# SinclaM/ray-tracer-challenge

Measured on AMD Instinct MI355X. Metric: Mrays/sec (primary+secondary), scenes/cover.json 1920x1080 depth 5, higher is better.
Workload: dtype f64

## Files before the change

ray-tracer-challenge_amd/csrc/rtc_capi.hip:

```cpp
#include <algorithm>
#include <chrono>
#include <atomic>
#include <cmath>
#include <cstdarg>
#include <cstdio>
#include <cstddef>
#include <cstring>
#include <memory>
#include <string>
#include <thread>
#include <unordered_set>
#include <vector>

#include "../../include/rtc.h"
#include "../../include/rtc_diag.h"
#include <sched.h>
#include <sys/mman.h>
#include <unistd.h>

#include "rtc_device.h"

extern "C" __global__ void rtc_scatter_tiles_kernel(const double* tiles, const uint32_t* tile_list, const uint32_t n_tiles, const uint32_t tile_w,
                                                    const uint32_t tile_h, const uint32_t hsize, const uint32_t vsize, double* canvas);
extern "C" __global__ void rtc_scatter_tiles_rgba8_kernel(const double* tiles, const uint32_t* tile_list, const uint32_t n_tiles,
// ... 226 lines not shown
  if (map.n_chunks >= min_chunks) return true;
  return simple3Trial(s, map) && threeWaves(s);
}

bool tablesInLds(const rtc_scene* s) {
  return s->dev.n_roots <= RTC_LDS_ROOTS && s->dev.n_materials <= RTC_LDS_MATERIALS &&
         s->dev.n_patterns <= RTC_LDS_PATTERNS && s->dev.n_lights <= RTC_LDS_LIGHTS;
}

struct KernelChoice {
  decltype(&rtc_render_kernel) fn;
  const char* name;
  decltype(&rtc_render_kernel_area) area = nullptr;
  decltype(&rtc_render_kernel_ms) ms = nullptr;
  decltype(&rtc_render_kernel_area_ms) area_ms = nullptr;
  KernelChoice(decltype(&rtc_render_kernel) f, const char* n) : fn(f), name(n) {}
  KernelChoice(decltype(&rtc_render_kernel_area) a, const char* n) : fn(nullptr), name(n), area(a) {}
  KernelChoice(decltype(&rtc_render_kernel_ms) m, const char* n) : fn(nullptr), name(n), ms(m) {}
  KernelChoice(decltype(&rtc_render_kernel_area_ms) am, const char* n) : fn(nullptr), name(n), area_ms(am) {}
  void launch(uint32_t blocks, hipStream_t stream, const rtc_scene* s, const DevScene& dev, const DevCamera& cam, const DevPixelMap& map,
              uint32_t max_depth, double* d_out, DevStats* st_now, DevStats* st_next) const {
    DevSampling smp = s->sampling;
    smp.pixel_base = static_cast<unsigned long long>(smp.sample_base) * (static_cast<unsigned long long>(cam.hsize) * cam.vsize);
    if (area_ms)
      hipLaunchKernelGGL(area_ms, dim3(blocks), dim3(256), 0, stream, dev, cam, map, max_depth, d_out, st_now, st_next, s->area, smp);
    else if (ms)
      hipLaunchKernelGGL(ms, dim3(blocks), dim3(256), 0, stream, dev, cam, map, max_depth, d_out, st_now, st_next, smp);
    else if (area)
      hipLaunchKernelGGL(area, dim3(blocks), dim3(256), 0, stream, dev, cam, map, max_depth, d_out, st_now, st_next, s->area);
    else
      hipLaunchKernelGGL(fn, dim3(blocks), dim3(256), 0, stream, dev, cam, map, max_depth, d_out, st_now, st_next);
  }
};
bool samplingKernels(const rtc_scene* s) { return s->sampling_on || s->sample_pass != 0u || rtcOptions().sampling_kernels != 0.0; }
#define RTC_KERNEL(k) KernelChoice{k, #k}
bool usesGeneral3(const rtc_scene* s) {
#if RTC_BVH8
  if (!s->general3_ok) return false;
  const double forced = rtcOptions().waves3;
  if (forced >= 0.0) return forced != 0.0;
  return threeWaves(s);
#else
  (void)s;
  return false;
#endif
}
KernelChoice ldsKernel(const rtc_scene* s, const DevPixelMap& map) {
  if (usesSimple3(s, map)) return s->box_cull ? RTC_KERNEL(rtc_render_kernel_simple3_b) : RTC_KERNEL(rtc_render_kernel_simple3);
#if RTC_BVH8
  if (usesGeneral3(s)) return RTC_KERNEL(rtc_render_kernel3);
#endif
  if (s->simple_kernel)
    return s->ext_kernel ? RTC_KERNEL(rtc_render_kernel_simple_ext) : (s->box_cull ? RTC_KERNEL(rtc_render_kernel_simple_b) : RTC_KERNEL(rtc_render_kernel_simple));
  if (s->flat_kernel) return s->ext_kernel ? RTC_KERNEL(rtc_render_kernel_flat_ext) : RTC_KERNEL(rtc_render_kernel_flat);
// ... 2572 lines not shown
```

ray-tracer-challenge_amd/csrc/rtc_device.h:

```cpp
#pragma once
#include <hip/hip_runtime.h>
#include <stdint.h>

#define RTC_NODE_BIT 0x80000000u
#define RTC_NO_LEAF 0xFFFFFFFFu
#define RTC_NO_ITEM 0xFFFFFFFFu
#define RTC_PACKET_ITEMS 16u
#define RTC_ITEM_MAX_CHUNKS 0x100000u

#ifndef RTC_TRAV_STACK
#define RTC_TRAV_STACK 64
#endif
#ifndef RTC_LDS_TRAV
#define RTC_LDS_TRAV 8
#endif
#ifndef RTC_MAX_DEPTH
#define RTC_MAX_DEPTH 16
#endif
#define RTC_RAY_STACK (RTC_MAX_DEPTH + 2)

struct DevMaterial {
  double ambient, diffuse, specular, shininess, reflective, transparency, ior;
  uint32_t pattern;
  uint32_t shininess_int;
// ... 209 lines not shown
};

struct DevPixelMap {
  uint32_t mode;
  uint32_t x0, y0, w, h;
  uint32_t tile_w, tile_h, first_tile, tile_stride, n_my_tiles;
  uint32_t tiles_x;
  uint32_t chunks_x;
  uint32_t chunks_per_region;
  uint32_t n_chunks;
  const uint32_t* __restrict__ tile_list;
  uint32_t n_units;
  const uint32_t* __restrict__ order;
  const uint32_t* __restrict__ n_units_dev;
  uint32_t* __restrict__ cost;
  uint32_t* __restrict__ packet_time;
  PendingRec* __restrict__ ray_stack;
  uint32_t ray_stack_levels;
#ifdef RTC_PROFILE
  uint32_t ray_stack_waves;
#endif
  uint32_t pull_min_idle;
  uint32_t row_packets;
};

struct DevChunkShape {
  float rays;
  float depth;
  uint32_t parts;
  uint8_t q[16];
};

struct DevSchedInfo {
  uint32_t n_units;
  uint32_t heaviest;
  uint32_t pad_[2];
  unsigned long long total;
};

#define RTC_PACK_CLASSES 136
struct DevPackState {
  uint32_t cnt[RTC_PACK_CLASSES];
  uint32_t cursor[RTC_PACK_CLASSES];
  unsigned long long total;
  uint32_t heaviest;
  uint32_t parts_cursor;
// ... 34 lines not shown
```

ray-tracer-challenge_amd/csrc/rtc_kernels.hip:

```cpp
#include "rtc_device.h"

#include <type_traits>

#if defined(RTC_PROFILE) && defined(RTC_PROFILE_LITE)
#define RTC_STAMP(sec)                                                     \
  do {                                                                     \
    if ((sec) == 7) prof_t = __builtin_amdgcn_s_memtime();                 \
    (void)prof_sec;                                                        \
  } while (0)
#define RTC_COUNT(slot) do { } while (0)
#define RTC_HIST_BEGIN() do { } while (0)
#define RTC_HIST_END(kind) do { } while (0)
#elif defined(RTC_PROFILE)
#define RTC_STAMP(sec)                                                     \
  do {                                                                     \
    const unsigned long long now_ = __builtin_amdgcn_s_memtime();          \
    prof_acc[prof_sec] += now_ - prof_t;                                   \
    prof_t = now_;                                                         \
    prof_sec = (sec);                                                      \
  } while (0)
#define RTC_COUNT(slot)                                                                 \
  do {                                                                                  \
    prof2[slot] += 1ull;                                                                \
    prof2[(slot) + 1] += static_cast<unsigned long long>(__builtin_popcountll(__ballot(true))); \
// ... 1863 lines not shown
  } else {
    pix_x = row_pt(cam.inv + 0, world_x, world_y, -1.0);
    pix_y = row_pt(cam.inv + 4, world_x, world_y, -1.0);
    pix_z = row_pt(cam.inv + 8, world_x, world_y, -1.0);
    r.ox = row_pt(cam.inv + 0, 0.0, 0.0, 0.0);
    r.oy = row_pt(cam.inv + 4, 0.0, 0.0, 0.0);
    r.oz = row_pt(cam.inv + 8, 0.0, 0.0, 0.0);
  }
  double dx = pix_x - r.ox, dy = pix_y - r.oy, dz = pix_z - r.oz;
  const double mag = __builtin_sqrt((dx * dx + dy * dy) + dz * dz);
  if (mag != 0.0) {
    dx = dx / mag;
    dy = dy / mag;
    dz = dz / mag;
  }
  r.dx = dx;
  r.dy = dy;
  r.dz = dz;
  return r;
}
#define RTC_SAMPLE_MASK 0xFFFFu
#define RTC_SAMPLE_OWNER 0x10000u

}

template <bool LDS, bool CSG, int WORLD = 0, int WAVES = 2, bool COOP = false, bool BOX = true, bool AREA = false, bool MS = false>
__device__ __forceinline__ void render_body(const DevScene& S, const DevCamera& cam, const DevPixelMap& map,
                                            const uint32_t max_depth, double* __restrict__ out,
                                            DevStats* __restrict__ stats, DevStats* __restrict__ next_stats,
                                            const DevAreaLights& area = DevAreaLights{}, const DevSampling& smp = DevSampling{}) {
  static_assert(!AREA || !COOP, "the area kernels run no cooperative iterations");
  static_assert(!MS || !COOP, "the sampling kernels run no cooperative iterations");
  RTC_PRIO_PHASE(RTC_PRIO_WORK);
#ifndef RTC_PROFILE
  if (blockIdx.x == 0u) {
    uint32_t* z = reinterpret_cast<uint32_t*>(next_stats);
    for (uint32_t i = threadIdx.x; i < sizeof(DevStats) / sizeof(uint32_t); i += blockDim.x) z[i] = 0u;
  }
#else
  (void)next_stats;
  if (threadIdx.x == 0u) rtc_prof_stats = stats;
#ifndef RTC_PROFILE_LITE
  if (threadIdx.x < 160u) rtc_prof_counts[threadIdx.x / 40u][threadIdx.x % 40u] = 0ull;
#endif
  __syncthreads();
#endif
// ... 82 lines not shown
    __syncthreads();
    recs = lds_recs;
    cull.sphere = lds_cull;
    cull.box = lds_box;
    mats = lds_mat;
    pats = lds_pat;
    lights = lds_light;
  }
#ifdef RTC_PROFILE
  if (!LDS) {
    if (threadIdx.x == 0u) {
      rtc_oob_avail[0] = S.n_root_recs;
      rtc_oob_avail[1] = S.n_root_cull;
      rtc_oob_avail[2] = S.n_root_box;
      rtc_oob_avail[3] = S.n_materials;
      rtc_oob_avail[4] = S.n_patterns;
      rtc_oob_avail[5] = 6u * S.n_lights;
    }
    __syncthreads();
  }
  const size_t out_extent = map.mode == 0u ? static_cast<size_t>(map.w) * map.h : static_cast<size_t>(map.n_my_tiles) * map.tile_w * map.tile_h;
  const bool stack_ok = (static_cast<size_t>(blockIdx.x) * 4u + (threadIdx.x >> 6)) < map.ray_stack_waves;
#endif
  const uint32_t lane = threadIdx.x & 63u;
  const unsigned long long lanes_below = (1ull << lane) - 1ull;
  auto bits_below = [&](unsigned long long m) -> uint32_t { return static_cast<uint32_t>(__builtin_popcountll(m & lanes_below)); };

  uint32_t items = RTC_NO_ITEM, item_next = RTC_PACKET_ITEMS;
  uint32_t pk_cur = RTC_NO_ITEM;
  unsigned long long pk_t0 = 0ull;
  const uint32_t n_units = map.n_units_dev != nullptr ? __builtin_amdgcn_readfirstlane(*map.n_units_dev) : map.n_units;
  uint32_t chunk_pos = 64u, chunk_end = 64u;
  uint32_t chunk_rx0 = 0u, chunk_ry0 = 0u, chunk_px0 = 0u, chunk_py0 = 0u, chunk_w = 0u, chunk_h = 0u;
  size_t chunk_out0 = 0;
  bool drained = false;
  bool first_pull = true;

  bool has_pixel = false, have_cur = false;
  bool shared = false;
  size_t out_index = 0;
  uint32_t share_rays = 0u;
  double* const acc = lds_acc[threadIdx.x >> 6][threadIdx.x & 63u];
  uint32_t* const trav_stack = FLAT ? nullptr : &lds_trav[threadIdx.x >> 6][0][(RTC_BVH8 ? 2u : 1u) * (threadIdx.x & 63u)];
  acc[0] = acc[1] = acc[2] = 0.0;
  uint32_t* samp_word = nullptr;
  if constexpr (MS) {
// ... 42 lines not shown
  const unsigned long long prof_real0 = __builtin_amdgcn_s_memrealtime();
  unsigned long long prof_real_fetch = prof_real0;
#endif
  for (;;) {
    RTC_STAMP(0);
    RTC_PRIO_PHASE(RTC_PRIO_DEAL);
    bool next_sample = false;
    if (!have_cur) {
      if (sp > base) {
        cur = load_level(--sp, lane);
        have_cur = true;
      } else {
        sp = base = 0;
        if constexpr (MS) {
          if (has_pixel) {
            const uint32_t w = *samp_word;
            if ((w & RTC_SAMPLE_OWNER) != 0u && (w & RTC_SAMPLE_MASK) + 1u < smp.samples) {
              *samp_word = w + 1u;
              next_sample = true;
            }
          }
        }
        if (!next_sample && has_pixel && RTC_IN_BOUNDS(RTC_OOB_CANVAS, out_index < out_extent)) {
          double* __restrict__ o = out + 3 * out_index;
          const double acc_r = acc[0], acc_g = acc[1], acc_b = acc[2];
          if (!shared) {
            typedef double Double2 __attribute__((ext_vector_type(2), aligned(8)));
            Double2 rg;
            rg.x = acc_r;
            rg.y = acc_g;
            __builtin_nontemporal_store(rg, reinterpret_cast<Double2*>(o));
            __builtin_nontemporal_store(acc_b, o + 2);
          } else
          {
            atomicAdd(o + 0, acc_r);
            atomicAdd(o + 1, acc_g);
            atomicAdd(o + 2, acc_b);
          }
          if (map.cost != nullptr) {
            if (!shared) {
              map.cost[out_index] = share_rays;
            } else {
              atomicAdd(map.cost + out_index, share_rays);
            }
          }
          share_rays = 0u;
          has_pixel = false;
        }
#ifdef RTC_PROFILE
        else if (has_pixel && !next_sample) {
          share_rays = 0u;
          has_pixel = false;
        }
#endif
      }
    }
    RTC_STAMP(8);
    {
      const bool idle = !have_cur && !next_sample;
      const bool donor = have_cur && sp > base;
      const unsigned long long imask = __ballot(idle), dmask = __ballot(donor);
      if (imask != 0ull && dmask != 0ull) {
        const uint32_t pairs = min(static_cast<uint32_t>(__builtin_popcountll(imask)),
                                   static_cast<uint32_t>(__builtin_popcountll(dmask)));
        const uint32_t irank = bits_below(imask);
        const uint32_t drank = bits_below(dmask);
        if (donor && drank < pairs) {
          mailbox[drank] = uint4{MS ? lane | (*samp_word & RTC_SAMPLE_MASK) << 8 : lane, static_cast<uint32_t>(base++), static_cast<uint32_t>(out_index), static_cast<uint32_t>(out_index >> 32)};
          if (!shared && RTC_IN_BOUNDS(RTC_OOB_CANVAS, out_index < out_extent)) {
            double* __restrict__ o = out + 3 * out_index;
            o[0] = 0.0;
            o[1] = 0.0;
            o[2] = 0.0;
            if (map.cost != nullptr) map.cost[out_index] = 0u;
            __builtin_amdgcn_fence(__ATOMIC_RELEASE, "workgroup");
          }
          shared = true;
        }
        __builtin_amdgcn_fence(__ATOMIC_RELEASE, "wavefront");
        __builtin_amdgcn_wave_barrier();
        __builtin_amdgcn_fence(__ATOMIC_ACQUIRE, "wavefront");
        if (idle && irank < pairs) {
          const uint4 m = mailbox[irank];
          cur = load_level(static_cast<int>(m.y), MS ? m.x & 63u : m.x);
          if constexpr (MS) *samp_word = m.x >> 8;
          out_index = static_cast<size_t>(m.z) | (static_cast<size_t>(m.w) << 32);
          have_cur = true;
          has_pixel = true;
          shared = true;
          acc[0] = acc[1] = acc[2] = 0.0;
          n_stolen++;
        }
        if (sp == base) sp = base = 0;
      }
    }
    RTC_STAMP(9);
    bool want = !have_cur && !next_sample, got_pixel = false;
    uint32_t new_px = 0u, new_py = 0u;
    unsigned long long wmask = __ballot(want);
    while (wmask) {
      if (chunk_pos >= chunk_end) {
        uint32_t unit = RTC_NO_ITEM;
        if (item_next < RTC_PACKET_ITEMS) unit = __builtin_amdgcn_readlane(items, item_next);
        RTC_STAMP(9);
        if (unit == RTC_NO_ITEM) {
          if (drained) break;
          if (static_cast<uint32_t>(__builtin_popcountll(wmask)) < map.pull_min_idle && __any(have_cur || got_pixel)) break;
          if (map.packet_time != nullptr && pk_cur != RTC_NO_ITEM) {
            if (lane == 0u) map.packet_time[pk_cur] = static_cast<uint32_t>((__builtin_amdgcn_s_memtime() - pk_t0) >> 4);
            pk_cur = RTC_NO_ITEM;
          }
          uint32_t c = 0u;
          RTC_STAMP(14);
          if (first_pull) {
            first_pull = false;
            c = blockIdx.x * 4u + (threadIdx.x >> 6);
          } else if (lane == 0u) {
            c = atomicAdd(&stats->next_chunk, 1u) + gridDim.x * 4u;
          }
          c = __builtin_amdgcn_readfirstlane(c);
          RTC_STAMP(15);
          if (c >= n_units) {
            drained = true;
            break;
          }
#ifdef RTC_PROFILE
          prof_last_unit = c;
          prof_first_unit = static_cast<unsigned>((__builtin_amdgcn_s_memtime() - prof_start) >> 8);
          prof_units += 1ull;
          prof_real_fetch = __builtin_amdgcn_s_memrealtime();
          for (int i = 0; i < 16; ++i) prof_snap[i] = prof_acc[i];
          prof_snap[7] = prof_iters;
#endif
          pk_cur = c;
          pk_t0 = __builtin_amdgcn_s_memtime();
          if (map.order != nullptr) {
            items = lane < RTC_PACKET_ITEMS ? map.order[static_cast<size_t>(c) * RTC_PACKET_ITEMS + lane] : RTC_NO_ITEM;
          } else {
            items = lane == 0u ? c : RTC_NO_ITEM;
          }
          item_next = 0u;
          continue;
        }
        item_next++;
        const bool rows = map.order == nullptr && map.row_packets != 0u;
        const uint32_t c = map.order != nullptr ? (unit & 0xFFFFFu) : (rows ? unit >> 3 : unit);
        chunk_pos = map.order != nullptr ? ((unit >> 20) & 63u) : (rows ? (unit & 7u) * 8u : 0u);
        chunk_end = map.order != nullptr ? chunk_pos + (unit >> 26) + 1u : (rows ? chunk_pos + 8u : 64u);
        const uint32_t region = c / map.chunks_per_region;
        const uint32_t cr = c - region * map.chunks_per_region;
        const uint32_t ccy = cr / map.chunks_x;
        chunk_rx0 = (cr - ccy * map.chunks_x) * 8u;
        chunk_ry0 = ccy * 8u;
        if (map.mode == 0u) {
          chunk_px0 = map.x0;
          chunk_py0 = map.y0;
          chunk_w = map.w;
          chunk_h = map.h;
          chunk_out0 = 0;
        } else {
          const uint32_t tile = map.mode == 1u ? map.first_tile + region * map.tile_stride : map.tile_list[region];
          const uint32_t ty = tile / map.tiles_x;
          chunk_px0 = (tile - ty * map.tiles_x) * map.tile_w;
          chunk_py0 = ty * map.tile_h;
          chunk_w = map.tile_w;
          chunk_h = map.tile_h;
          chunk_out0 = static_cast<size_t>(region) * map.tile_h * map.tile_w;
        }
      }
      const uint32_t avail = chunk_end - chunk_pos;
      const uint32_t rank = bits_below(wmask);
      if (want && rank < avail) {
        const uint32_t k = chunk_pos + rank;
        const uint32_t rx = chunk_rx0 + (k & 7u), ry = chunk_ry0 + (k >> 3);
        const bool in_buffer = rx < chunk_w && ry < chunk_h;
        const uint32_t px = chunk_px0 + rx, py = chunk_py0 + ry;
        if (in_buffer && px < cam.hsize && py < cam.vsize) {
          new_px = px;
          new_py = py;
          got_pixel = true;
          want = false;
          out_index = chunk_out0 + static_cast<size_t>(ry) * chunk_w + rx;
        }
      }
      chunk_pos += min(avail, static_cast<uint32_t>(__builtin_popcountll(wmask)));
      wmask = __ballot(want);
    }
    if constexpr (MS) {
      if (got_pixel || next_sample) {
        uint32_t k = 0u;
        if (next_sample) {
          k = *samp_word & RTC_SAMPLE_MASK;
          map_pixel(map, out_index, new_px, new_py);
        } else {
          *samp_word = RTC_SAMPLE_OWNER;
          shared = false;
          acc[0] = acc[1] = acc[2] = 0.0;
        }
        cur.ray = camera_sample(cam, smp, new_px, new_py, k);
        cur.weight = smp.weight;
        cur.remaining = max_depth;
        have_cur = true;
        has_pixel = true;
        n_primary++;
      }
    } else if (got_pixel) {
      const double xoffset = (static_cast<double>(new_px) + 0.5) * cam.pixel_size;
      const double yoffset = (static_cast<double>(new_py) + 0.5) * cam.pixel_size;
      const double world_x = cam.half_width - xoffset;
      const double world_y = cam.half_height - yoffset;
      const double pix_x = row_pt(cam.inv + 0, world_x, world_y, -1.0);
      const double pix_y = row_pt(cam.inv + 4, world_x, world_y, -1.0);
      const double pix_z = row_pt(cam.inv + 8, world_x, world_y, -1.0);
      cur.ray.ox = row_pt(cam.inv + 0, 0.0, 0.0, 0.0);
      cur.ray.oy = row_pt(cam.inv + 4, 0.0, 0.0, 0.0);
      cur.ray.oz = row_pt(cam.inv + 8, 0.0, 0.0, 0.0);
      double dx = pix_x - cur.ray.ox, dy = pix_y - cur.ray.oy, dz = pix_z - cur.ray.oz;
      const double mag = __builtin_sqrt((dx * dx + dy * dy) + dz * dz);
      if (mag != 0.0) {
        dx = dx / mag;
        dy = dy / mag;
        dz = dz / mag;
      }
      cur.ray.dx = dx;
      cur.ray.dy = dy;
      cur.ray.dz = dz;
      cur.weight = 1.0;
      cur.remaining = max_depth;
      have_cur = true;
      has_pixel = true;
      shared = false;
      acc[0] = acc[1] = acc[2] = 0.0;
      n_primary++;
    }
    if (!__any(have_cur)) break;
    struct Yield {
      double contrib[3] = {0.0, 0.0, 0.0};
      Pending kid_now, kid_later;
      uint32_t n_kids = 0u, share = 0u, secondary = 0u, shadow_calls = 0u, shadow_traced = 0u, overflow = 0u;
// ... 214 lines not shown
      }
      RTC_STAMP(12);
      const bool shadow_matters = !(mat.diffuse == 0.0 && mat.specular == 0.0);
      const bool deal_lights = COOP && coop && S.n_lights <= 2u;
      const uint32_t li_first = deal_lights ? (member >> 2) : 0u, li_step = deal_lights ? 2u : 1u;
      const uint32_t s_member = deal_lights ? (member & 3u) : member, s_stride = deal_lights ? 4u : stride;
      const unsigned calls_before = it_shadow_calls, traced_before = it_shadow_traced, share_before = it_share;
      for (uint32_t li = li_first; li < S.n_lights; li += li_step) {
#ifdef RTC_PROFILE
        if (!RTC_IN_BOUNDS(RTC_OOB_LIGHTS, 6u * li + 6u <= RTC_AVAIL(5))) continue;
        if (AREA && !RTC_IN_BOUNDS(RTC_OOB_LIGHTS, RTC_AREA_ROW * li + RTC_AREA_ROW <= area_avail)) continue;
#endif
        if constexpr (AREA) {
          const double* __restrict__ A = area_rows + static_cast<size_t>(RTC_AREA_ROW) * li;
          const unsigned long long bits = static_cast<unsigned long long>(__double_as_longlong(A[12]));
          if ((bits >> RTC_AREA_KIND_BIT) & 1ull) {
            const uint32_t us = static_cast<uint32_t>(bits) & ((1u << RTC_AREA_STEP_BITS) - 1u);
            const uint32_t vs = static_cast<uint32_t>(bits >> RTC_AREA_STEP_BITS) & ((1u << RTC_AREA_STEP_BITS) - 1u);
            const bool jitter = (bits >> RTC_AREA_JITTER_BIT) & 1ull;
            const uint32_t n_samples = us * vs;
            it_shadow_calls += n_samples;
            unsigned long long pixel = 0ull;
            if (jitter) {
              uint32_t px, py;
              if (map.mode == 0u) {
                const uint32_t ry = static_cast<uint32_t>(out_index / map.w);
                px = map.x0 + static_cast<uint32_t>(out_index - static_cast<size_t>(ry) * map.w);
                py = map.y0 + ry;
              } else {
                const size_t per_tile = static_cast<size_t>(map.tile_w) * map.tile_h;
                const uint32_t region = static_cast<uint32_t>(out_index / per_tile);
                const uint32_t r = static_cast<uint32_t>(out_index - static_cast<size_t>(region) * per_tile);
                const uint32_t ry = r / map.tile_w, rx = r - ry * map.tile_w;
                const uint32_t tile = map.mode == 1u ? map.first_tile + region * map.tile_stride : map.tile_list[region];
                const uint32_t ty = tile / map.tiles_x;
                px = (tile - ty * map.tiles_x) * map.tile_w + rx;
                py = ty * map.tile_h + ry;
              }
              pixel = static_cast<unsigned long long>(py) * cam.hsize + px;
              if constexpr (MS) pixel = pixel * smp.samples + (*samp_word & RTC_SAMPLE_MASK) + smp.pixel_base;
            }
            auto to_sample = [&](uint32_t u, uint32_t v, double& vx, double& vy, double& vz) {
              double ju = 0.5, jv = 0.5;
              if (jitter) {
                const uint32_t k = v * us + u;
                ju = rtc_area_jitter(area.seed, pixel, S.n_lights, li, k, 0u);
                jv = rtc_area_jitter(area.seed, pixel, S.n_lights, li, k, 1u);
              }
              const double fu = static_cast<double>(u) + ju, fv = static_cast<double>(v) + jv;
              vx = ((A[0] + A[3] * fu) + A[6] * fv) - ovx;
              vy = ((A[1] + A[4] * fu) + A[7] * fv) - ovy;
              vz = ((A[2] + A[5] * fu) + A[8] * fv) - ovz;
            };
            const double er = color.r * A[9], eg = color.g * A[10], eb = color.b * A[11];
            const double ka = mat.ambient;
            double lr_ = er * ka, lg_ = eg * ka, lb_ = eb * ka;
            double dr = 0.0, dg = 0.0, db = 0.0;
            if (shadow_matters) {
              for (uint32_t v = 0u; v < vs; ++v)
                for (uint32_t u = 0u; u < us; ++u) {
                  double vx, vy, vz;
                  to_sample(u, v, vx, vy, vz);
// ... 246 lines not shown
        acc[0] += yield.contrib[0];
        acc[1] += yield.contrib[1];
        acc[2] += yield.contrib[2];
        share_rays += yield.share;
        n_secondary += yield.secondary;
        n_shadow_calls += yield.shadow_calls;
        n_shadow_traced += yield.shadow_traced;
        overflow |= yield.overflow;
        if (yield.n_kids == 2u) {
          if (sp < stack_cap) {
            push_level(sp++, yield.kid_later);
          } else {
            overflow = CSG ? (overflow | 1u) : 1u;
          }
        }
        if (yield.n_kids != 0u) {
          cur = yield.kid_now;
          have_cur = true;
        }
      }
    }
  }

  if (map.packet_time != nullptr && pk_cur != RTC_NO_ITEM && lane == 0u)
    map.packet_time[pk_cur] = static_cast<uint32_t>((__builtin_amdgcn_s_memtime() - pk_t0) >> 4);
#ifdef RTC_PROFILE
  RTC_STAMP(7);
  prof_acc[7] = prof_iters;
  if (lane == 0u) {
    for (int i = 0; i < 16; ++i) atomicAdd(&stats->prof[i], prof_acc[i]);
    atomicMin(&stats->prof_t0, prof_t - prof_start);
    atomicMax(&stats->prof_t1, ((prof_t - prof_start) << 24) | (prof_last_unit & 0xFFFFFFull));
    atomicAdd(&stats->prof_busy, prof_t - prof_start);
    for (int i = 0; i < 8; ++i) atomicAdd(&stats->prof2[i], prof2[i]);
    for (int i = 0; i < 21; ++i) atomicAdd(&stats->prof3[i], prof3[i]);
#ifndef RTC_PROFILE_LITE
    for (int i = 0; i < 8; ++i) {
      atomicAdd(&stats->prof4[i], rtc_prof_counts[threadIdx.x >> 6][i]);
      atomicAdd(&stats->prof5[i], rtc_prof_counts[threadIdx.x >> 6][8 + i]);
    }
    for (int i = 0; i < 24; ++i) atomicAdd(&stats->prof6[i], rtc_prof_counts[threadIdx.x >> 6][16 + i]);
#endif
    const unsigned wid = (blockIdx.x * 4u + (threadIdx.x >> 6)) & 4095u;
    stats->prof_log[wid][0] = prof_t - prof_start;
    stats->prof_log[wid][1] = prof_iters;
    stats->prof_log[wid][2] = prof_units;
    stats->prof_log[wid][3] = (static_cast<unsigned long long>(prof_first_unit) << 32) | prof_last_unit;
    for (int i = 0; i < 16; ++i) stats->prof_last[wid][i] = prof_acc[i] - prof_snap[i];
#ifdef RTC_PROFILE_LITE
    stats->prof_last[wid][0] = prof_real0;
    stats->prof_last[wid][1] = __builtin_amdgcn_s_memrealtime();
    stats->prof_last[wid][2] = prof_real_fetch;
#endif
  }
#endif
  {
    __shared__ unsigned long long wg_sum[6];
    if (threadIdx.x < 6u) wg_sum[threadIdx.x] = 0ull;
    __syncthreads();
    const unsigned long long s_pri = wave_sum(n_primary), s_sec = wave_sum(n_secondary), s_shc = wave_sum(n_shadow_calls),
                             s_sht = wave_sum(n_shadow_traced), s_ovf = wave_sum(CSG ? (overflow != 0u ? 1u : 0u) : overflow), s_stolen = wave_sum(n_stolen);
    if constexpr (CSG)
    if (__any((overflow >> 8) != 0u)) {
      unsigned need = overflow >> 8;
      for (int off = 32; off > 0; off >>= 1) need = max(need, static_cast<unsigned>(__shfl_xor(need, off, 64)));
      if (lane == 0u) atomicMax(&stats->csg_needed, need);
    }
    if (lane == 0u) {
      atomicAdd(&wg_sum[0], s_pri);
      atomicAdd(&wg_sum[1], s_sec);
      atomicAdd(&wg_sum[2], s_shc);
      atomicAdd(&wg_sum[3], s_sht);
      if (s_ovf) atomicAdd(&wg_sum[4], s_ovf);
      if (s_stolen) atomicAdd(&wg_sum[5], s_stolen);
    }
    __syncthreads();
    if (threadIdx.x == 0u) {
      atomicAdd(&stats->primary, wg_sum[0]);
      atomicAdd(&stats->secondary, wg_sum[1]);
      atomicAdd(&stats->shadow_calls, wg_sum[2]);
      atomicAdd(&stats->shadow_traced, wg_sum[3]);
      if (wg_sum[4]) atomicAdd(&stats->overflow, wg_sum[4]);
      if (wg_sum[5]) atomicAdd(&stats->stolen, static_cast<unsigned int>(wg_sum[5]));
    }
  }
}

extern "C" __global__ void __launch_bounds__(256, RTC_LB2)
rtc_render_kernel(const DevScene S, const DevCamera cam, const DevPixelMap map, const uint32_t max_depth,
                  double* __restrict__ out, DevStats* __restrict__ stats, DevStats* __restrict__ next_stats) {
  render_body<true, false>(S, cam, map, max_depth, out, stats, next_stats);
}

extern "C" __global__ void __launch_bounds__(256, RTC_LB2)
rtc_render_kernel_bigworld(const DevScene S, const DevCamera cam, const DevPixelMap map, const uint32_t max_depth,
                           double* __restrict__ out, DevStats* __restrict__ stats, DevStats* __restrict__ next_stats) {
  render_body<false, false>(S, cam, map, max_depth, out, stats, next_stats);
}

extern "C" __global__ void __launch_bounds__(256, RTC_LB2)
rtc_render_kernel_simple(const DevScene S, const DevCamera cam, const DevPixelMap map, const uint32_t max_depth,
                         double* __restrict__ out, DevStats* __restrict__ stats, DevStats* __restrict__ next_stats) {
  render_body<true, false, 2, 2, true, false>(S, cam, map, max_depth, out, stats, next_stats);
}

extern "C" __global__ void __launch_bounds__(256, RTC_LB2)
rtc_render_kernel_simple_b(const DevScene S, const DevCamera cam, const DevPixelMap map, const uint32_t max_depth,
                           double* __restrict__ out, DevStats* __restrict__ stats, DevStats* __restrict__ next_stats) {
  render_body<true, false, 2, 2, true, true>(S, cam, map, max_depth, out, stats, next_stats);
}

extern "C" __global__ void __launch_bounds__(256, 3)
rtc_render_kernel_simple3(const DevScene S, const DevCamera cam, const DevPixelMap map, const uint32_t max_depth,
                          double* __restrict__ out, DevStats* __restrict__ stats, DevStats* __restrict__ next_stats) {
  render_body<true, false, 2, 3, false, false>(S, cam, map, max_depth, out, stats, next_stats);
}

extern "C" __global__ void __launch_bounds__(256, 3)
rtc_render_kernel_simple3_b(const DevScene S, const DevCamera cam, const DevPixelMap map, const uint32_t max_depth,
                            double* __restrict__ out, DevStats* __restrict__ stats, DevStats* __restrict__ next_stats) {
  render_body<true, false, 2, 3, false, true>(S, cam, map, max_depth, out, stats, next_stats);
}

#if RTC_BVH8
extern "C" __global__ void __launch_bounds__(256, 3)
rtc_render_kernel3(const DevScene S, const DevCamera cam, const DevPixelMap map, const uint32_t max_depth,
                   double* __restrict__ out, DevStats* __restrict__ stats, DevStats* __restrict__ next_stats) {
  render_body<true, false, 0, 3>(S, cam, map, max_depth, out, stats, next_stats);
}
#endif

extern "C" __global__ void __launch_bounds__(256, RTC_LB2)
rtc_render_kernel_ext(const DevScene S, const DevCamera cam, const DevPixelMap map, const uint32_t max_depth,
                      double* __restrict__ out, DevStats* __restrict__ stats, DevStats* __restrict__ next_stats) {
  render_body<true, true>(S, cam, map, max_depth, out, stats, next_stats);
}

extern "C" __global__ void __launch_bounds__(256, RTC_LB2)
rtc_render_kernel_simple_ext(const DevScene S, const DevCamera cam, const DevPixelMap map, const uint32_t max_depth,
                             double* __restrict__ out, DevStats* __restrict__ stats, DevStats* __restrict__ next_stats) {
  render_body<true, true, 2, 2, false, false>(S, cam, map, max_depth, out, stats, next_stats);
}

extern "C" __global__ void __launch_bounds__(256, RTC_LB2)
rtc_render_kernel_flat(const DevScene S, const DevCamera cam, const DevPixelMap map, const uint32_t max_depth,
                       double* __restrict__ out, DevStats* __restrict__ stats, DevStats* __restrict__ next_stats) {
  render_body<true, false, 1>(S, cam, map, max_depth, out, stats, next_stats);
}

extern "C" __global__ void __launch_bounds__(256, RTC_LB2)
rtc_render_kernel_flat_ext(const DevScene S, const DevCamera cam, const DevPixelMap map, const uint32_t max_depth,
                           double* __restrict__ out, DevStats* __restrict__ stats, DevStats* __restrict__ next_stats) {
  render_body<true, true, 1>(S, cam, map, max_depth, out, stats, next_stats);
}

extern "C" __global__ void __launch_bounds__(256, RTC_LB2)
rtc_render_kernel_bigworld_ext(const DevScene S, const DevCamera cam, const DevPixelMap map, const uint32_t max_depth,
                               double* __restrict__ out, DevStats* __restrict__ stats, DevStats* __restrict__ next_stats) {
  render_body<false, true>(S, cam, map, max_depth, out, stats, next_stats);
}

extern "C" __global__ void __launch_bounds__(256, RTC_LB2)
rtc_render_kernel_area(const DevScene S, const DevCamera cam, const DevPixelMap map, const uint32_t max_depth,
                       double* __restrict__ out, DevStats* __restrict__ stats, DevStats* __restrict__ next_stats,
                       const DevAreaLights area) {
  render_body<true, true, 0, 2, false, true, true>(S, cam, map, max_depth, out, stats, next_stats, area);
}

extern "C" __global__ void __launch_bounds__(256, RTC_LB2)
rtc_render_kernel_area_bigworld(const DevScene S, const DevCamera cam, const DevPixelMap map, const uint32_t max_depth,
                                double* __restrict__ out, DevStats* __restrict__ stats, DevStats* __restrict__ next_stats,
                                const DevAreaLights area) {
  render_body<false, true, 0, 2, false, true, true>(S, cam, map, max_depth, out, stats, next_stats, area);
}

extern "C" __global__ void __launch_bounds__(256, RTC_LB2)
rtc_render_kernel_ms(const DevScene S, const DevCamera cam, const DevPixelMap map, const uint32_t max_depth,
                     double* __restrict__ out, DevStats* __restrict__ stats, DevStats* __restrict__ next_stats,
                     const DevSampling smp) {
  render_body<true, true, 0, 2, false, true, false, true>(S, cam, map, max_depth, out, stats, next_stats, DevAreaLights{}, smp);
}

extern "C" __global__ void __launch_bounds__(256, RTC_LB2)
rtc_render_kernel_ms_bigworld(const DevScene S, const DevCamera cam, const DevPixelMap map, const uint32_t max_depth,
                              double* __restrict__ out, DevStats* __restrict__ stats, DevStats* __restrict__ next_stats,
                              const DevSampling smp) {
  render_body<false, true, 0, 2, false, true, false, true>(S, cam, map, max_depth, out, stats, next_stats, DevAreaLights{}, smp);
}

extern "C" __global__ void __launch_bounds__(256, RTC_LB2)
rtc_render_kernel_area_ms(const DevScene S, const DevCamera cam, const DevPixelMap map, const uint32_t max_depth,
                          double* __restrict__ out, DevStats* __restrict__ stats, DevStats* __restrict__ next_stats,
                          const DevAreaLights area, const DevSampling smp) {
  render_body<true, true, 0, 2, false, true, true, true>(S, cam, map, max_depth, out, stats, next_stats, area, smp);
}

extern "C" __global__ void __launch_bounds__(256, RTC_LB2)
rtc_render_kernel_area_ms_bigworld(const DevScene S, const DevCamera cam, const DevPixelMap map, const uint32_t max_depth,
// ... 539 lines not shown
        const uint32_t G = min((m * a / (a + b)) / a, (m - m * a / (a + b)) / b);
        const uint32_t sa = G * a, sb = G * b;
        if (r < sa) {
          rank = keep + (r / a) * (a + b) + r % a;
        } else if (r >= m - sb) {
          const uint32_t c = m - 1u - r;
          rank = keep + (c / b) * (a + b) + a + c % b;
        } else {
          rank = keep + G * (a + b) + (r - sa);
        }
      }
    }
  }
  const uint32_t p = state->parts_cursor + rank;
  const uint32_t have = min(kk, state->cnt[k] - j);
  uint32_t items[RTC_PACKET_ITEMS];
#pragma unroll
  for (uint32_t q = 0; q < RTC_PACKET_ITEMS; ++q)
    items[q] = q < have ? ((sorted[i + q] & 0xFFFFFu) | (63u << 26)) : RTC_NO_ITEM;
  uint4* row = reinterpret_cast<uint4*>(order_out + static_cast<size_t>(p) * RTC_PACKET_ITEMS);
#pragma unroll
  for (uint32_t q = 0; q < RTC_PACKET_ITEMS / 4u; ++q) row[q] = uint4{items[q * 4u], items[q * 4u + 1u], items[q * 4u + 2u], items[q * 4u + 3u]};
}
```

Baseline: 15660.

## Reload cold kernel args from kernarg segment and precompute divisor reciprocals

For most render kernel variants, rarely used arguments (camera, pixel map, output and stats pointers) are re-read from the kernarg segment pointer at each use. This avoids keeping them live in scalar registers across the long traversal loop, with the aim of lowering register pressure. The host now precomputes reciprocals so the chunk and tile integer divisions become a multiply-high plus one correction step. The kernels are also split across two translation units, one for the general variants and one for the rest, which changes how each is compiled. The cost is extra scalar loads at each use and an asm barrier that stops the compiler from caching these values.

```diff
diff --git a/ray-tracer-challenge_amd/csrc/rtc_capi.hip b/ray-tracer-challenge_amd/csrc/rtc_capi.hip
--- a/ray-tracer-challenge_amd/csrc/rtc_capi.hip
+++ b/ray-tracer-challenge_amd/csrc/rtc_capi.hip
@@ -272,14 +272,19 @@
               uint32_t max_depth, double* d_out, DevStats* st_now, DevStats* st_next) const {
     DevSampling smp = s->sampling;
     smp.pixel_base = static_cast<unsigned long long>(smp.sample_base) * (static_cast<unsigned long long>(cam.hsize) * cam.vsize);
+    DevPixelMap m = map;
+    auto rcp = [](uint32_t d) { return d != 0u ? 0xFFFFFFFFu / d : 0u; };
+    m.chunks_per_region_rcp = rcp(m.chunks_per_region);
+    m.chunks_x_rcp = rcp(m.chunks_x);
+    m.tiles_x_rcp = rcp(m.tiles_x);
     if (area_ms)
-      hipLaunchKernelGGL(area_ms, dim3(blocks), dim3(256), 0, stream, dev, cam, map, max_depth, d_out, st_now, st_next, s->area, smp);
+      hipLaunchKernelGGL(area_ms, dim3(blocks), dim3(256), 0, stream, dev, cam, m, max_depth, d_out, st_now, st_next, s->area, smp);
     else if (ms)
-      hipLaunchKernelGGL(ms, dim3(blocks), dim3(256), 0, stream, dev, cam, map, max_depth, d_out, st_now, st_next, smp);
+      hipLaunchKernelGGL(ms, dim3(blocks), dim3(256), 0, stream, dev, cam, m, max_depth, d_out, st_now, st_next, smp);
     else if (area)
-      hipLaunchKernelGGL(area, dim3(blocks), dim3(256), 0, stream, dev, cam, map, max_depth, d_out, st_now, st_next, s->area);
+      hipLaunchKernelGGL(area, dim3(blocks), dim3(256), 0, stream, dev, cam, m, max_depth, d_out, st_now, st_next, s->area);
     else
-      hipLaunchKernelGGL(fn, dim3(blocks), dim3(256), 0, stream, dev, cam, map, max_depth, d_out, st_now, st_next);
+      hipLaunchKernelGGL(fn, dim3(blocks), dim3(256), 0, stream, dev, cam, m, max_depth, d_out, st_now, st_next);
   }
 };
 bool samplingKernels(const rtc_scene* s) { return s->sampling_on || s->sample_pass != 0u || rtcOptions().sampling_kernels != 0.0; }
diff --git a/ray-tracer-challenge_amd/csrc/rtc_device.h b/ray-tracer-challenge_amd/csrc/rtc_device.h
--- a/ray-tracer-challenge_amd/csrc/rtc_device.h
+++ b/ray-tracer-challenge_amd/csrc/rtc_device.h
@@ -255,6 +255,7 @@
 #endif
   uint32_t pull_min_idle;
   uint32_t row_packets;
+  uint32_t chunks_per_region_rcp, chunks_x_rcp, tiles_x_rcp;
 };
 
 struct DevChunkShape {
diff --git a/ray-tracer-challenge_amd/csrc/rtc_kernels.hip b/ray-tracer-challenge_amd/csrc/rtc_kernels.hip
--- a/ray-tracer-challenge_amd/csrc/rtc_kernels.hip
+++ b/ray-tracer-challenge_amd/csrc/rtc_kernels.hip
@@ -1,4 +1,8 @@
 #include "rtc_device.h"
+
+#ifndef RTC_KERNELS_GENERAL
+#define RTC_KERNELS_GENERAL 0
+#endif
 
 #include <type_traits>
 
@@ -1909,6 +1913,43 @@
 #define RTC_SAMPLE_MASK 0xFFFFu
 #define RTC_SAMPLE_OWNER 0x10000u
 
+struct RenderArgs {
+  DevScene S;
+  DevCamera cam;
+  DevPixelMap map;
+  uint32_t max_depth;
+  double* out;
+  DevStats* stats;
+  DevStats* next_stats;
+};
+__device__ __forceinline__ const RenderArgs* cold_args() {
+  typedef const __attribute__((address_space(4))) RenderArgs* KernargPtr;
+  KernargPtr a = (KernargPtr)__builtin_amdgcn_kernarg_segment_ptr();
+  asm volatile("" : "+s"(a));
+  return (const RenderArgs*)a;
+}
+struct FetchArgs {
+  const DevCamera& cam;
+  const DevPixelMap& map;
+  double* out;
+  DevStats* stats;
+};
+template <bool COLD>
+__device__ __forceinline__ FetchArgs fetch_args(const DevCamera& cam, const DevPixelMap& map, double* out, DevStats* stats) {
+  if constexpr (COLD) {
+    const RenderArgs* const a = cold_args();
+    return {a->cam, a->map, a->out, a->stats};
+  } else {
+    return {cam, map, out, stats};
+  }
+}
+
+__device__ __forceinline__ uint32_t div_by(uint32_t n, uint32_t d, uint32_t r) {
+  uint32_t q = __umulhi(n, r);
+  if (n - q * d >= d) ++q;
+  return q;
+}
+
 }
 
 template <bool LDS, bool CSG, int WORLD = 0, int WAVES = 2, bool COOP = false, bool BOX = true, bool AREA = false, bool MS = false>
@@ -2037,6 +2078,7 @@
   const size_t out_extent = map.mode == 0u ? static_cast<size_t>(map.w) * map.h : static_cast<size_t>(map.n_my_tiles) * map.tile_w * map.tile_h;
   const bool stack_ok = (static_cast<size_t>(blockIdx.x) * 4u + (threadIdx.x >> 6)) < map.ray_stack_waves;
 #endif
+  constexpr bool COLD_ARGS = !(LDS && CSG && WORLD == 0 && !AREA && !MS) && !(WORLD == 2 && WAVES == 3 && !BOX);
   const uint32_t lane = threadIdx.x & 63u;
   const unsigned long long lanes_below = (1ull << lane) - 1ull;
   auto bits_below = [&](unsigned long long m) -> uint32_t { return static_cast<uint32_t>(__builtin_popcountll(m & lanes_below)); };
@@ -2125,7 +2167,8 @@
           }
         }
         if (!next_sample && has_pixel && RTC_IN_BOUNDS(RTC_OOB_CANVAS, out_index < out_extent)) {
-          double* __restrict__ o = out + 3 * out_index;
+          const FetchArgs args = fetch_args<COLD_ARGS>(cam, map, out, stats);
+          double* __restrict__ o = args.out + 3 * out_index;
           const double acc_r = acc[0], acc_g = acc[1], acc_b = acc[2];
           if (!shared) {
             typedef double Double2 __attribute__((ext_vector_type(2), aligned(8)));
@@ -2140,11 +2183,11 @@
             atomicAdd(o + 1, acc_g);
             atomicAdd(o + 2, acc_b);
           }
-          if (map.cost != nullptr) {
+          if (args.map.cost != nullptr) {
             if (!shared) {
-              map.cost[out_index] = share_rays;
+              args.map.cost[out_index] = share_rays;
             } else {
-              atomicAdd(map.cost + out_index, share_rays);
+              atomicAdd(args.map.cost + out_index, share_rays);
             }
           }
           share_rays = 0u;
@@ -2171,11 +2214,12 @@
         if (donor && drank < pairs) {
           mailbox[drank] = uint4{MS ? lane | (*samp_word & RTC_SAMPLE_MASK) << 8 : lane, static_cast<uint32_t>(base++), static_cast<uint32_t>(out_index), static_cast<uint32_t>(out_index >> 32)};
           if (!shared && RTC_IN_BOUNDS(RTC_OOB_CANVAS, out_index < out_extent)) {
-            double* __restrict__ o = out + 3 * out_index;
+            const FetchArgs args = fetch_args<COLD_ARGS>(cam, map, out, stats);
+            double* __restrict__ o = args.out + 3 * out_index;
             o[0] = 0.0;
             o[1] = 0.0;
             o[2] = 0.0;
-            if (map.cost != nullptr) map.cost[out_index] = 0u;
+            if (args.map.cost != nullptr) args.map.cost[out_index] = 0u;
             __builtin_amdgcn_fence(__ATOMIC_RELEASE, "workgroup");
           }
           shared = true;
@@ -2203,14 +2247,15 @@
     unsigned long long wmask = __ballot(want);
     while (wmask) {
       if (chunk_pos >= chunk_end) {
+        const FetchArgs args = fetch_args<COLD_ARGS>(cam, map, out, stats);
         uint32_t unit = RTC_NO_ITEM;
         if (item_next < RTC_PACKET_ITEMS) unit = __builtin_amdgcn_readlane(items, item_next);
         RTC_STAMP(9);
         if (unit == RTC_NO_ITEM) {
           if (drained) break;
-          if (static_cast<uint32_t>(__builtin_popcountll(wmask)) < map.pull_min_idle && __any(have_cur || got_pixel)) break;
-          if (map.packet_time != nullptr && pk_cur != RTC_NO_ITEM) {
-            if (lane == 0u) map.packet_time[pk_cur] = static_cast<uint32_t>((__builtin_amdgcn_s_memtime() - pk_t0) >> 4);
+          if (static_cast<uint32_t>(__builtin_popcountll(wmask)) < args.map.pull_min_idle && __any(have_cur || got_pixel)) break;
+          if (args.map.packet_time != nullptr && pk_cur != RTC_NO_ITEM) {
+            if (lane == 0u) args.map.packet_time[pk_cur] = static_cast<uint32_t>((__builtin_amdgcn_s_memtime() - pk_t0) >> 4);
             pk_cur = RTC_NO_ITEM;
           }
           uint32_t c = 0u;
@@ -2219,7 +2264,7 @@
             first_pull = false;
             c = blockIdx.x * 4u + (threadIdx.x >> 6);
           } else if (lane == 0u) {
-            c = atomicAdd(&stats->next_chunk, 1u) + gridDim.x * 4u;
+            c = atomicAdd(&args.stats->next_chunk, 1u) + gridDim.x * 4u;
           }
           c = __builtin_amdgcn_readfirstlane(c);
           RTC_STAMP(15);
@@ -2237,8 +2282,8 @@
 #endif
           pk_cur = c;
           pk_t0 = __builtin_amdgcn_s_memtime();
-          if (map.order != nullptr) {
-            items = lane < RTC_PACKET_ITEMS ? map.order[static_cast<size_t>(c) * RTC_PACKET_ITEMS + lane] : RTC_NO_ITEM;
+          if (args.map.order != nullptr) {
+            items = lane < RTC_PACKET_ITEMS ? args.map.order[static_cast<size_t>(c) * RTC_PACKET_ITEMS + lane] : RTC_NO_ITEM;
           } else {
             items = lane == 0u ? c : RTC_NO_ITEM;
           }
@@ -2246,39 +2291,41 @@
           continue;
         }
         item_next++;
-        const bool rows = map.order == nullptr && map.row_packets != 0u;
-        const uint32_t c = map.order != nullptr ? (unit & 0xFFFFFu) : (rows ? unit >> 3 : unit);
-        chunk_pos = map.order != nullptr ? ((unit >> 20) & 63u) : (rows ? (unit & 7u) * 8u : 0u);
-        chunk_end = map.order != nullptr ? chunk_pos + (unit >> 26) + 1u : (rows ? chunk_pos + 8u : 64u);
-        const uint32_t region = c / map.chunks_per_region;
-        const uint32_t cr = c - region * map.chunks_per_region;
-        const uint32_t ccy = cr / map.chunks_x;
-        chunk_rx0 = (cr - ccy * map.chunks_x) * 8u;
+        const bool rows = args.map.order == nullptr && args.map.row_packets != 0u;
+        const uint32_t c = args.map.order != nullptr ? (unit & 0xFFFFFu) : (rows ? unit >> 3 : unit);
+        chunk_pos = args.map.order != nullptr ? ((unit >> 20) & 63u) : (rows ? (unit & 7u) * 8u : 0u);
+        chunk_end = args.map.order != nullptr ? chunk_pos + (unit >> 26) + 1u : (rows ? chunk_pos + 8u : 64u);
+        const uint32_t region = COLD_ARGS ? div_by(c, args.map.chunks_per_region, args.map.chunks_per_region_rcp)
+                                          : c / args.map.chunks_per_region;
+        const uint32_t cr = c - region * args.map.chunks_per_region;
+        const uint32_t ccy = COLD_ARGS ? div_by(cr, args.map.chunks_x, args.map.chunks_x_rcp) : cr / args.map.chunks_x;
+        chunk_rx0 = (cr - ccy * args.map.chunks_x) * 8u;
         chunk_ry0 = ccy * 8u;
-        if (map.mode == 0u) {
-          chunk_px0 = map.x0;
-          chunk_py0 = map.y0;
-          chunk_w = map.w;
-          chunk_h = map.h;
+        if (args.map.mode == 0u) {
+          chunk_px0 = args.map.x0;
+          chunk_py0 = args.map.y0;
+          chunk_w = args.map.w;
+          chunk_h = args.map.h;
           chunk_out0 = 0;
         } else {
-          const uint32_t tile = map.mode == 1u ? map.first_tile + region * map.tile_stride : map.tile_list[region];
-          const uint32_t ty = tile / map.tiles_x;
-          chunk_px0 = (tile - ty * map.tiles_x) * map.tile_w;
-          chunk_py0 = ty * map.tile_h;
-          chunk_w = map.tile_w;
-          chunk_h = map.tile_h;
-          chunk_out0 = static_cast<size_t>(region) * map.tile_h * map.tile_w;
+          const uint32_t tile = args.map.mode == 1u ? args.map.first_tile + region * args.map.tile_stride : args.map.tile_list[region];
+          const uint32_t ty = COLD_ARGS ? div_by(tile, args.map.tiles_x, args.map.tiles_x_rcp) : tile / args.map.tiles_x;
+          chunk_px0 = (tile - ty * args.map.tiles_x) * args.map.tile_w;
+          chunk_py0 = ty * args.map.tile_h;
+          chunk_w = args.map.tile_w;
+          chunk_h = args.map.tile_h;
+          chunk_out0 = static_cast<size_t>(region) * args.map.tile_h * args.map.tile_w;
         }
       }
       const uint32_t avail = chunk_end - chunk_pos;
       const uint32_t rank = bits_below(wmask);
       if (want && rank < avail) {
+        const FetchArgs args = fetch_args<COLD_ARGS>(cam, map, out, stats);
         const uint32_t k = chunk_pos + rank;
         const uint32_t rx = chunk_rx0 + (k & 7u), ry = chunk_ry0 + (k >> 3);
         const bool in_buffer = rx < chunk_w && ry < chunk_h;
         const uint32_t px = chunk_px0 + rx, py = chunk_py0 + ry;
-        if (in_buffer && px < cam.hsize && py < cam.vsize) {
+        if (in_buffer && px < args.cam.hsize && py < args.cam.vsize) {
           new_px = px;
           new_py = py;
           got_pixel = true;
@@ -2291,16 +2338,17 @@
     }
     if constexpr (MS) {
       if (got_pixel || next_sample) {
+        const FetchArgs args = fetch_args<COLD_ARGS>(cam, map, out, stats);
         uint32_t k = 0u;
         if (next_sample) {
           k = *samp_word & RTC_SAMPLE_MASK;
-          map_pixel(map, out_index, new_px, new_py);
+          map_pixel(args.map, out_index, new_px, new_py);
         } else {
           *samp_word = RTC_SAMPLE_OWNER;
           shared = false;
           acc[0] = acc[1] = acc[2] = 0.0;
         }
-        cur.ray = camera_sample(cam, smp, new_px, new_py, k);
+        cur.ray = camera_sample(args.cam, smp, new_px, new_py, k);
         cur.weight = smp.weight;
         cur.remaining = max_depth;
         have_cur = true;
@@ -2308,16 +2356,17 @@
         n_primary++;
       }
     } else if (got_pixel) {
-      const double xoffset = (static_cast<double>(new_px) + 0.5) * cam.pixel_size;
-      const double yoffset = (static_cast<double>(new_py) + 0.5) * cam.pixel_size;
-      const double world_x = cam.half_width - xoffset;
-      const double world_y = cam.half_height - yoffset;
-      const double pix_x = row_pt(cam.inv + 0, world_x, world_y, -1.0);
-      const double pix_y = row_pt(cam.inv + 4, world_x, world_y, -1.0);
-      const double pix_z = row_pt(cam.inv + 8, world_x, world_y, -1.0);
-      cur.ray.ox = row_pt(cam.inv + 0, 0.0, 0.0, 0.0);
-      cur.ray.oy = row_pt(cam.inv + 4, 0.0, 0.0, 0.0);
-      cur.ray.oz = row_pt(cam.inv + 8, 0.0, 0.0, 0.0);
+      const FetchArgs args = fetch_args<COLD_ARGS>(cam, map, out, stats);
+      const double xoffset = (static_cast<double>(new_px) + 0.5) * args.cam.pixel_size;
+      const double yoffset = (static_cast<double>(new_py) + 0.5) * args.cam.pixel_size;
+      const double world_x = args.cam.half_width - xoffset;
+      const double world_y = args.cam.half_height - yoffset;
+      const double pix_x = row_pt(args.cam.inv + 0, world_x, world_y, -1.0);
+      const double pix_y = row_pt(args.cam.inv + 4, world_x, world_y, -1.0);
+      const double pix_z = row_pt(args.cam.inv + 8, world_x, world_y, -1.0);
+      cur.ray.ox = row_pt(args.cam.inv + 0, 0.0, 0.0, 0.0);
+      cur.ray.oy = row_pt(args.cam.inv + 4, 0.0, 0.0, 0.0);
+      cur.ray.oz = row_pt(args.cam.inv + 8, 0.0, 0.0, 0.0);
       double dx = pix_x - cur.ray.ox, dy = pix_y - cur.ray.oy, dz = pix_z - cur.ray.oz;
       const double mag = __builtin_sqrt((dx * dx + dy * dy) + dz * dz);
       if (mag != 0.0) {
@@ -2578,22 +2627,23 @@
             it_shadow_calls += n_samples;
             unsigned long long pixel = 0ull;
             if (jitter) {
+              const FetchArgs args = fetch_args<COLD_ARGS>(cam, map, out, stats);
               uint32_t px, py;
-              if (map.mode == 0u) {
-                const uint32_t ry = static_cast<uint32_t>(out_index / map.w);
-                px = map.x0 + static_cast<uint32_t>(out_index - static_cast<size_t>(ry) * map.w);
-                py = map.y0 + ry;
+              if (args.map.mode == 0u) {
+                const uint32_t ry = static_cast<uint32_t>(out_index / args.map.w);
+                px = args.map.x0 + static_cast<uint32_t>(out_index - static_cast<size_t>(ry) * args.map.w);
+                py = args.map.y0 + ry;
               } else {
-                const size_t per_tile = static_cast<size_t>(map.tile_w) * map.tile_h;
+                const size_t per_tile = static_cast<size_t>(args.map.tile_w) * args.map.tile_h;
                 const uint32_t region = static_cast<uint32_t>(out_index / per_tile);
                 const uint32_t r = static_cast<uint32_t>(out_index - static_cast<size_t>(region) * per_tile);
-                const uint32_t ry = r / map.tile_w, rx = r - ry * map.tile_w;
-                const uint32_t tile = map.mode == 1u ? map.first_tile + region * map.tile_stride : map.tile_list[region];
-                const uint32_t ty = tile / map.tiles_x;
-                px = (tile - ty * map.tiles_x) * map.tile_w + rx;
-                py = ty * map.tile_h + ry;
+                const uint32_t ry = r / args.map.tile_w, rx = r - ry * args.map.tile_w;
+                const uint32_t tile = args.map.mode == 1u ? args.map.first_tile + region * args.map.tile_stride : args.map.tile_list[region];
+                const uint32_t ty = tile / args.map.tiles_x;
+                px = (tile - ty * args.map.tiles_x) * args.map.tile_w + rx;
+                py = ty * args.map.tile_h + ry;
               }
-              pixel = static_cast<unsigned long long>(py) * cam.hsize + px;
+              pixel = static_cast<unsigned long long>(py) * args.cam.hsize + px;
               if constexpr (MS) pixel = pixel * smp.samples + (*samp_word & RTC_SAMPLE_MASK) + smp.pixel_base;
             }
             auto to_sample = [&](uint32_t u, uint32_t v, double& vx, double& vy, double& vz) {
@@ -2886,8 +2936,11 @@
     }
   }
 
-  if (map.packet_time != nullptr && pk_cur != RTC_NO_ITEM && lane == 0u)
-    map.packet_time[pk_cur] = static_cast<uint32_t>((__builtin_amdgcn_s_memtime() - pk_t0) >> 4);
+  if (pk_cur != RTC_NO_ITEM && lane == 0u) {
+    const FetchArgs args = fetch_args<COLD_ARGS>(cam, map, out, stats);
+    if (args.map.packet_time != nullptr)
+      args.map.packet_time[pk_cur] = static_cast<uint32_t>((__builtin_amdgcn_s_memtime() - pk_t0) >> 4);
+  }
 #ifdef RTC_PROFILE
   RTC_STAMP(7);
   prof_acc[7] = prof_iters;
@@ -2919,6 +2972,7 @@
   }
 #endif
   {
+    const FetchArgs args = fetch_args<COLD_ARGS>(cam, map, out, stats);
     __shared__ unsigned long long wg_sum[6];
     if (threadIdx.x < 6u) wg_sum[threadIdx.x] = 0ull;
     __syncthreads();
@@ -2928,7 +2982,7 @@
     if (__any((overflow >> 8) != 0u)) {
       unsigned need = overflow >> 8;
       for (int off = 32; off > 0; off >>= 1) need = max(need, static_cast<unsigned>(__shfl_xor(need, off, 64)));
-      if (lane == 0u) atomicMax(&stats->csg_needed, need);
+      if (lane == 0u) atomicMax(&args.stats->csg_needed, need);
     }
     if (lane == 0u) {
       atomicAdd(&wg_sum[0], s_pri);
@@ -2940,16 +2994,17 @@
     }
     __syncthreads();
     if (threadIdx.x == 0u) {
-      atomicAdd(&stats->primary, wg_sum[0]);
-      atomicAdd(&stats->secondary, wg_sum[1]);
-      atomicAdd(&stats->shadow_calls, wg_sum[2]);
-      atomicAdd(&stats->shadow_traced, wg_sum[3]);
-      if (wg_sum[4]) atomicAdd(&stats->overflow, wg_sum[4]);
-      if (wg_sum[5]) atomicAdd(&stats->stolen, static_cast<unsigned int>(wg_sum[5]));
-    }
-  }
-}
-
+      atomicAdd(&args.stats->primary, wg_sum[0]);
+      atomicAdd(&args.stats->secondary, wg_sum[1]);
+      atomicAdd(&args.stats->shadow_calls, wg_sum[2]);
+      atomicAdd(&args.stats->shadow_traced, wg_sum[3]);
+      if (wg_sum[4]) atomicAdd(&args.stats->overflow, wg_sum[4]);
+      if (wg_sum[5]) atomicAdd(&args.stats->stolen, static_cast<unsigned int>(wg_sum[5]));
+    }
+  }
+}
+
+#if RTC_KERNELS_GENERAL
 extern "C" __global__ void __launch_bounds__(256, RTC_LB2)
 rtc_render_kernel(const DevScene S, const DevCamera cam, const DevPixelMap map, const uint32_t max_depth,
                   double* __restrict__ out, DevStats* __restrict__ stats, DevStats* __restrict__ next_stats) {
@@ -2962,6 +3017,9 @@
   render_body<false, false>(S, cam, map, max_depth, out, stats, next_stats);
 }
 
+#endif
+
+#if !RTC_KERNELS_GENERAL
 extern "C" __global__ void __launch_bounds__(256, RTC_LB2)
 rtc_render_kernel_simple(const DevScene S, const DevCamera cam, const DevPixelMap map, const uint32_t max_depth,
                          double* __restrict__ out, DevStats* __restrict__ stats, DevStats* __restrict__ next_stats) {
@@ -2985,7 +3043,9 @@
                             double* __restrict__ out, DevStats* __restrict__ stats, DevStats* __restrict__ next_stats) {
   render_body<true, false, 2, 3, false, true>(S, cam, map, max_depth, out, stats, next_stats);
 }
-
+#endif
+
+#if RTC_KERNELS_GENERAL
 #if RTC_BVH8
 extern "C" __global__ void __launch_bounds__(256, 3)
 rtc_render_kernel3(const DevScene S, const DevCamera cam, const DevPixelMap map, const uint32_t max_depth,
@@ -3000,6 +3060,9 @@
   render_body<true, true>(S, cam, map, max_depth, out, stats, next_stats);
 }
 
+#endif
+
+#if !RTC_KERNELS_GENERAL
 extern "C" __global__ void __launch_bounds__(256, RTC_LB2)
 rtc_render_kernel_simple_ext(const DevScene S, const DevCamera cam, const DevPixelMap map, const uint32_t max_depth,
                              double* __restrict__ out, DevStats* __restrict__ stats, DevStats* __restrict__ next_stats) {
@@ -3017,7 +3080,9 @@
                            double* __restrict__ out, DevStats* __restrict__ stats, DevStats* __restrict__ next_stats) {
   render_body<true, true, 1>(S, cam, map, max_depth, out, stats, next_stats);
 }
-
+#endif
+
+#if RTC_KERNELS_GENERAL
 extern "C" __global__ void __launch_bounds__(256, RTC_LB2)
 rtc_render_kernel_bigworld_ext(const DevScene S, const DevCamera cam, const DevPixelMap map, const uint32_t max_depth,
                                double* __restrict__ out, DevStats* __restrict__ stats, DevStats* __restrict__ next_stats) {
@@ -3038,6 +3103,9 @@
   render_body<false, true, 0, 2, false, true, true>(S, cam, map, max_depth, out, stats, next_stats, area);
 }
 
+#endif
+
+#if !RTC_KERNELS_GENERAL
 extern "C" __global__ void __launch_bounds__(256, RTC_LB2)
 rtc_render_kernel_ms(const DevScene S, const DevCamera cam, const DevPixelMap map, const uint32_t max_depth,
                      double* __restrict__ out, DevStats* __restrict__ stats, DevStats* __restrict__ next_stats,
@@ -3623,3 +3691,4 @@
 #pragma unroll
   for (uint32_t q = 0; q < RTC_PACKET_ITEMS / 4u; ++q) row[q] = uint4{items[q * 4u], items[q * 4u + 1u], items[q * 4u + 2u], items[q * 4u + 3u]};
 }
+#endif
diff --git a/ray-tracer-challenge_amd/csrc/rtc_kernels_general.hip b/ray-tracer-challenge_amd/csrc/rtc_kernels_general.hip
--- /dev/null
+++ b/ray-tracer-challenge_amd/csrc/rtc_kernels_general.hip
@@ -0,0 +1,2 @@
+#define RTC_KERNELS_GENERAL 1
+#include "rtc_kernels.hip"
```

New measurement: 15930 (median of 6 runs). 1.8% higher.
